# jianwen-xie/Latent-Space-Normalizing-Flow

Measured on AMD Instinct MI355X. Metric: latent-samples/sec through flow+logdet, nz=128 B=65536, higher is better.
Workload: dtype bf16x3; 1 GPU; CIFAR-10 flow prior nz=128 f_width=64 f_depth=5 affine, forward+logdet+log-prob, B=65536 synthetic z per evaluation (BASELINE.json configs[2]); rows_per_gpu=65536, global_rows=65536, parallelism=single GPU, streams=3, clock_ramp_launches_before_warmup=600

## Files before the change

latent-space-normalizing-flow_amd/csrc/lsnf_fwd3p.hip:

```cpp
#include <stdlib.h>
#include <type_traits>
#include "lsnf_l16.h"
#include "lsnf_launch.h"

#if LSNF_L16_PARTS != 3
#error "lsnf_fwd3p.hip is the three-term bf16 kernel"
#endif

#ifndef LSNF_FILLMASK
#define LSNF_FILLMASK 0x7f
#endif

namespace {

struct Fwd3pArgs {
    const float* consts; const float* panels3;
    const float* z_in; const float* objective;
    float* z_out; float* logdet_out; float* ll_out;
    int B, nz, half, n_blocks, vec4;
    double* stats;
    float* hdump; int width;
    float* z_saved; float* act_saved;
    unsigned long long* stamps;
};

#ifdef LSNF_STAMPS
#define P_STAMP(i, INSN)                                                                                \
    do { __builtin_amdgcn_sched_barrier(0);                                                             \
         unsigned long long t_; asm volatile(INSN " %0\n\ts_waitcnt lgkmcnt(0)" : "=s"(t_) :: "memory");  \
         __builtin_amdgcn_sched_barrier(0);                                                             \
         if (a.stamps && lane == 0) a.stamps[(((size_t)blockIdx.x * NWAVES + wave) & 2047) * 64 + (i)] = t_; } while (0)
#else
#define P_STAMP(i, INSN) do {} while (0)
#endif

template <int WT_>
struct Fwd3pCfg : LsnfStackCfg<2, WT_> {
    using S = LsnfStackCfg<2, WT_>;
    static constexpr int F = LSNF_FRAG3_FLOATS;
    static constexpr int OFF3_S2 = F * S::P1 * S::KT1;
    static constexpr int OFF3_S3 = OFF3_S2 + F * S::P2 * S::KT2;
    static constexpr int OFF3_S4 = OFF3_S3 + F * S::P3 * S::KT3;
    static constexpr int BLOCK3 = OFF3_S4 + F * S::P4 * S::KT4;
    static constexpr int SLOT3 = 2 * S::MAXKT * F;
    static constexpr int CONST_FLOATS = S::FWD_CONST;
};

__device__ __forceinline__ void keep(unsigned a, unsigned b, unsigned c) { asm volatile("" :: "v"(a), "v"(b), "v"(c)); }
__device__ __forceinline__ void keep(float a, float b, float c, float d, float e) { asm volatile("" :: "v"(a), "v"(b), "v"(c), "v"(d), "v"(e)); }

struct StepDesc { int acc, tile, s, frag; };
template <int KT> constexpr StepDesc mkstep(int acc, int tl, int in_tile, int kt, int s) { return StepDesc{acc, in_tile, s, ((tl * KT + kt) * 2 + s) * 3}; }

struct Tile16 { f32x4v q[4]; };
struct SplitTile16 { unsigned d[2][3][4]; };

template <int HT, int ST>
__device__ __forceinline__ Tile16 load_tile16(int t, const float* __restrict__ z, const int* rows, int nz, int half, int g, int vw) {
    Tile16 x;
    const int hh = t / HT, tt = t % HT;
#pragma unroll
    for (int ft = 0; ft < 2; ++ft)
#pragma unroll
        for (int st = 0; st < ST; ++st) {
            const int f0 = 32 * tt + l16_feat0(ft, g), col0 = hh * half + f0, q = 2 * ft + st;
            const float* zr = z + (long)rows[st] * (long)nz;
            if (vw == 4) {
                f32x4 v = {0.f, 0.f, 0.f, 0.f};
                if (f0 < half) v = *reinterpret_cast<const f32x4*>(zr + col0);
                x.q[q][0] = v[0]; x.q[q][1] = v[1]; x.q[q][2] = v[2]; x.q[q][3] = v[3];
            } else if (vw == 2) {
                f32x2 v0 = {0.f, 0.f}, v1 = {0.f, 0.f};
                if (f0 < half) v0 = *reinterpret_cast<const f32x2*>(zr + col0);
                if (f0 + 2 < half) v1 = *reinterpret_cast<const f32x2*>(zr + col0 + 2);
                x.q[q][0] = v0[0]; x.q[q][1] = v0[1]; x.q[q][2] = v1[0]; x.q[q][3] = v1[1];
            } else {
#pragma unroll
                for (int j = 0; j < 4; ++j) x.q[q][j] = (f0 + j < half) ? zr[col0 + j] : 0.0f;
            }
        }
    return x;
}
template <int HT, int ST>
__device__ __forceinline__ void store_tile16(int t, const Tile16& x, float* __restrict__ z, const int* rows, const bool* live,
                                             int nz, int half, int g, int vw) {
    const int hh = t / HT, tt = t % HT;
#pragma unroll
    for (int ft = 0; ft < 2; ++ft)
#pragma unroll
        for (int st = 0; st < ST; ++st) {
            if (!live[st]) continue;
            const int f0 = 32 * tt + l16_feat0(ft, g), col0 = hh * half + f0, q = 2 * ft + st;
            float* zr = z + (long)rows[st] * (long)nz;
            if (vw == 4) {
                if (f0 < half) { f32x4 v = {x.q[q][0], x.q[q][1], x.q[q][2], x.q[q][3]}; *reinterpret_cast<f32x4*>(zr + col0) = v; }
            } else if (vw == 2) {
                if (f0 < half) { f32x2 v = {x.q[q][0], x.q[q][1]}; *reinterpret_cast<f32x2*>(zr + col0) = v; }
                if (f0 + 2 < half) { f32x2 v = {x.q[q][2], x.q[q][3]}; *reinterpret_cast<f32x2*>(zr + col0 + 2) = v; }
            } else {
#pragma unroll
                for (int j = 0; j < 4; ++j)
                    if (f0 + j < half) zr[col0 + j] = x.q[q][j];
            }
        }
}
__device__ __forceinline__ const float* bias_lane_ptr(const float* cb, int g) { return cb + (g & 1) * 16 + 4 * (g >> 1); }
__device__ __forceinline__ f32x4v bias_quad(const float* lane_ptr, int float_off) {
    const f32x4 v = *reinterpret_cast<const f32x4*>(lane_ptr + float_off);
    f32x4v r;
#pragma unroll
    for (int j = 0; j < 4; ++j) r[j] = v[j];
    return r;
}
template <class PH> constexpr bool first_touch(int i) {
    for (int j = 0; j < i; ++j)
        if (PH::at(j).acc == PH::at(i).acc && PH::at(j).s == PH::at(i).s) return false;
    return true;
}
template <int ST> __device__ __forceinline__ constexpr int unit_quad(int q) { return ST == 2 ? q : (q & ~1); }
template <int ST> __device__ __forceinline__ constexpr int unit_pair0(int q) { return ST == 2 ? 0 : (q & 1); }
template <int ST> __device__ __forceinline__ constexpr int unit_st(int q) { return ST == 2 ? (q & 1) : 0; }
template <bool RELU, int ST>
__device__ __forceinline__ void split_q16(const Tile16& x, int q, SplitTile16& out) {
#pragma clang fp contract(off)
    const int ft = q >> 1, st = unit_st<ST>(q), qr = unit_quad<ST>(q);
#pragma unroll
    for (int jj = 0; jj < ST; ++jj) {
        const int j = unit_pair0<ST>(q) + jj;
        float a = x.q[qr][2 * j], b = x.q[qr][2 * j + 1];
        if (RELU) { a = fmaxf(a, 0.0f); b = fmaxf(b, 0.0f); }
        const unsigned p1 = pk_bf16(a, b);
        a -= __builtin_bit_cast(float, p1 << 16); b -= __builtin_bit_cast(float, p1 & 0xffff0000u);
        const unsigned p2 = pk_bf16(a, b);
        a -= __builtin_bit_cast(float, p2 << 16); b -= __builtin_bit_cast(float, p2 & 0xffff0000u);
        const int d = 2 * ft + j;
        out.d[st][0][d] = p1; out.d[st][1][d] = p2; out.d[st][2][d] = pk_bf16(a, b);
        keep(out.d[st][0][d], out.d[st][1][d], out.d[st][2][d]);
    }
}
template <int ST>
__device__ __forceinline__ void sigmoid_q16(Tile16& p, int q, float* lsum ) {
    const int st = unit_st<ST>(q), qr = unit_quad<ST>(q), r0 = 2 * unit_pair0<ST>(q);
#pragma unroll
    for (int r = r0; r < r0 + 2 * ST; ++r) {
        float sig, l2;
        lsnf_sigmoid_log2(p.q[qr][r], sig, l2);
        p.q[qr][r] = sig; lsum[st] += l2;
    }
    keep(p.q[qr][r0], p.q[qr][r0 + 1], p.q[qr][r0 + 2 * ST - 2], p.q[qr][r0 + 2 * ST - 1], lsum[st]);
}
template <int ST>
__device__ __forceinline__ void couple_q16(Tile16& v, const Tile16& t, const Tile16& sig, int q) {
    const int qr = unit_quad<ST>(q), r0 = 2 * unit_pair0<ST>(q);
#pragma unroll
    for (int r = r0; r < r0 + 2 * ST; ++r) v.q[qr][r] = (v.q[qr][r] + t.q[qr][r]) * sig.q[qr][r];
}

#ifndef LSNF_STASH_AUX
#define LSNF_STASH_AUX 0
#endif
#ifndef LSNF_STASH_PARTS
#define LSNF_STASH_PARTS 7
#endif
typedef unsigned u32x4s __attribute__((ext_vector_type(4)));
struct StashLane { unsigned zoff, soff, moff, msh, hoff; };
struct StashRsrc { __amdgpu_buffer_rsrc_t r[2]; };
__device__ __forceinline__ StashRsrc stash_rsrc(const float* p, unsigned bytes, unsigned second_off) {
    char* c = reinterpret_cast<char*>(const_cast<float*>(p));
    return StashRsrc{{__builtin_amdgcn_make_buffer_rsrc(c, 0, (int)bytes, 0x00020000),
                      __builtin_amdgcn_make_buffer_rsrc(c + second_off, 0, (int)(bytes > second_off ? bytes - second_off : 0u), 0x00020000)}};
}
template <int HT>
__device__ __forceinline__ void stash_row_quad(const StashRsrc& rs, const StashLane& sl, int t, int q, const Tile16& x, int nz, int half, int g) {
    if constexpr (!(LSNF_STASH_PARTS & 4)) return;
    const int ft = q >> 1, st = q & 1, hh = t / HT, tt = t % HT;
    unsigned off = sl.zoff;
    if (st) off += (unsigned)(16 * nz * 4);
    off = (32 * tt + 16 * ft + 4 * g < half) ? off : 0x80000000u;
    const u32x4s v = __builtin_bit_cast(u32x4s, x.q[q]);
    __builtin_amdgcn_raw_buffer_store_b128(v, rs.r[hh], off + (unsigned)((32 * tt + 16 * ft) * 4), 0, LSNF_STASH_AUX);
}
__device__ __forceinline__ void stash_sigma_quad(const StashRsrc& rs, const StashLane& sl, int t, int q, const Tile16& sg) {
    if constexpr (!(LSNF_STASH_PARTS & 2)) return;
    const int ft = q >> 1, st = q & 1;
    const u32x4s v = __builtin_bit_cast(u32x4s, sg.q[q]);
    __builtin_amdgcn_raw_buffer_store_b128(v, rs.r[t], sl.soff + (unsigned)((2 * ft * 64 + 16 * st) * 16), 0, LSNF_STASH_AUX);
}
__device__ __forceinline__ void mask_q16(const Tile16& h, int q, unsigned (&mk)[2][2]) {
    if constexpr (!(LSNF_STASH_PARTS & 1)) return;
    unsigned m = 0;
#pragma unroll
    for (int r = 3; r >= 0; --r) m = __builtin_amdgcn_alignbit(m, __builtin_bit_cast(unsigned, 0.0f - h.q[q][r]), 31);
    mk[q & 1][q >> 1] = m;
    asm volatile("" :: "v"(m));
}
__device__ __forceinline__ void stash_mask_words(const StashRsrc& rs, const StashLane& sl, int tile, const unsigned (&mk)[2][2]) {
    if constexpr (!(LSNF_STASH_PARTS & 1)) return;
    const unsigned w0 = mk[0][0] | (mk[0][1] << 8), w1 = mk[1][0] | (mk[1][1] << 8);
    unsigned x = ((w0 << 16) | w1) << sl.msh;
    x = lsnf_pair_or32(x);
    __builtin_amdgcn_raw_buffer_store_b32(x >> 16, rs.r[0], sl.moff + (unsigned)(tile * 64 * 4), 0, 0);
    __builtin_amdgcn_raw_buffer_store_b32(x & 0xffffu, rs.r[0], sl.moff + (unsigned)((tile * 64 + 16) * 4), 0, 0);
}
__device__ __forceinline__ void stash_h_quad(const StashRsrc& rs, const StashLane& sl, int t, int q, const Tile16& h, int width) {
    const int ft = q >> 1, st = q & 1;
    f32x4v r;
#pragma unroll
    for (int j = 0; j < 4; ++j) r[j] = fmaxf(h.q[q][j], 0.0f);
    const unsigned off = (32 * t + 16 * ft < width) ? sl.hoff : 0x80000000u;
    __builtin_amdgcn_raw_buffer_store_b128(__builtin_bit_cast(u32x4s, r), rs.r[t], off + (unsigned)((ft * 2 + st) * 1024), 0, LSNF_STASH_AUX);
}

template <int NM, int NV>
__device__ __forceinline__ void pin_mfma() {
    lsnf_static_for<NM>([&](auto mc) {
        constexpr int m = decltype(mc)::value, V = NV / NM + (m < NV % NM ? 1 : 0);
        __builtin_amdgcn_sched_group_barrier(0x008, 1, 0);
        if constexpr (V > 0) __builtin_amdgcn_sched_group_barrier(0x402, V, 0);
    });
}
template <class PH, int ST, class Fill, class Mid>
__device__ __forceinline__ void run_phase16(Tile16* acc, const float* bias_ptr , const SplitTile16* in, const float* lbuf, int lane, Fill&& fill, Mid&& mid) {
    const bf16x8* wp = reinterpret_cast<const bf16x8*>(lbuf) + lane;
    __builtin_amdgcn_sched_barrier(0);
    bf16x8 a[3];
#pragma unroll
    for (int p = 0; p < 3; ++p) a[p] = wp[(PH::at(0).frag + p) * 64];
    f32x4v bq = bias_quad(bias_ptr, 32 * PH::btile(PH::at(0).acc) + 8 * PH::at(0).s);
    __builtin_amdgcn_sched_group_barrier(0x100, 4, 0);
    lsnf_static_for<PH::N>([&](auto ic) {
        constexpr int i = decltype(ic)::value;
        constexpr StepDesc d = PH::at(i);
        mid(ic);
        bf16x8 na[3];
        f32x4v nbq = bq;
#pragma unroll
        for (int p = 0; p < 3; ++p) na[p] = a[p];
        if constexpr (i + 1 < PH::N) {
#pragma unroll
            for (int p = 0; p < 3; ++p) na[p] = wp[(PH::at(i + 1).frag + p) * 64];
            if constexpr (first_touch<PH>(i + 1)) nbq = bias_quad(bias_ptr, 32 * PH::btile(PH::at(i + 1).acc) + 8 * PH::at(i + 1).s);
        }
#ifndef LSNF_ABL_NOFILL
        fill(ic);
#endif
        const SplitTile16& x = in[d.tile];
        constexpr bool first = first_touch<PH>(i);
#define LSNF_Q_MMA(WI, XI) \
        acc[d.acc].q[2 * d.s + 0] = __builtin_amdgcn_mfma_f32_16x16x32_bf16(a[WI], __builtin_bit_cast(bf16x8, u32x4{x.d[0][XI][0], x.d[0][XI][1], x.d[0][XI][2], x.d[0][XI][3]}), (first && WI == 2 && XI == 0) ? bq : acc[d.acc].q[2 * d.s + 0], 0, 0, 0); \
        if constexpr (ST == 2) acc[d.acc].q[2 * d.s + 1] = __builtin_amdgcn_mfma_f32_16x16x32_bf16(a[WI], __builtin_bit_cast(bf16x8, u32x4{x.d[1][XI][0], x.d[1][XI][1], x.d[1][XI][2], x.d[1][XI][3]}), (first && WI == 2 && XI == 0) ? bq : acc[d.acc].q[2 * d.s + 1], 0, 0, 0);
#ifdef LSNF_ABL_NOMFMA
        LSNF_Q_MMA(0, 0)
#else
        LSNF_F3_TERMS(LSNF_Q_MMA)
#endif
#undef LSNF_Q_MMA
        if constexpr (i + 1 < PH::N) __builtin_amdgcn_sched_group_barrier(0x100, first_touch<PH>(i + 1) ? 4 : 3, 0);
        pin_mfma<6 * ST, (PH::valu(i) * ST) / 2>();
        __builtin_amdgcn_sched_barrier(0);
#pragma unroll
        for (int p = 0; p < 3; ++p) a[p] = na[p];
        bq = nbq;
    });
}

struct QhNoStores { static constexpr int stores(int) { return 0; } };
struct QhS1a : QhNoStores {
    static constexpr int N = 16;
    static constexpr int btile(int acc) { return acc; }
    static constexpr StepDesc at(int i) { return mkstep<4>((i >> 1) & 1, (i >> 1) & 1, i >> 2, i >> 2, i & 1); }
    static constexpr int valu(int i) { return i < 2 ? 22 : (i < 6 ? 28 : (i < 8 ? 16 : (i < 12 ? 22 : 0))); }
};
struct QhS1b : QhNoStores {
    static constexpr int N = 16;
    static constexpr int btile(int acc) { return 2 + acc; }
    static constexpr StepDesc at(int i) { return mkstep<4>((i >> 1) & 1, (i >> 1) & 1, i >> 2, i >> 2, i & 1); }
    static constexpr int valu(int i) { return i >= 8 ? 22 : 0; }
};
struct QhS23 : QhNoStores {
    static constexpr int N = 16;
    static constexpr int btile(int acc) { return 4 + acc; }
    static constexpr StepDesc at(int i) {
        if (i < 8) { const int tl = i >> 2, kt = (i >> 1) & 1; return mkstep<2>(tl, tl, kt, kt, i & 1); }
        const int j = i - 8, kt = j >> 2, tl = (j >> 1) & 1;
        return mkstep<2>(2 + tl, 2 + tl, 2 + kt, kt, j & 1);
    }
    static constexpr int valu(int i) { return (i >= 4 && i < 12) ? 26 : (i >= 13 ? 26 : 0); }
};
struct QhS4 : QhNoStores {
    static constexpr int N = 16;
    static constexpr int btile(int acc) { return 8 + (acc == 0 ? 2 : (acc == 1 ? 0 : (acc == 2 ? 3 : 1))); }
    static constexpr int torder(int j) { return j == 0 ? 2 : (j == 1 ? 0 : (j == 2 ? 3 : 1)); }
    static constexpr StepDesc at(int i) { const int kt = i >> 3, j = (i >> 1) & 3; return mkstep<2>(j, torder(j), kt, kt, i & 1); }
    static constexpr int valu(int i) { return i < 4 ? 26 : (i < 9 ? 0 : (i < 12 ? 28 : (i == 12 ? 36 : (i == 13 ? 24 : 22)))); }
};

struct QsS1a : QhS1a {
    static constexpr int valu(int i) { return (i == 6 || i == 7) ? 20 : (i >= 8 && i < 12 ? 23 : QhS1a::valu(i)); }
    static constexpr int stores(int i) { return (i >= 2 && i < 6) ? 1 : ((i == 6 || i == 7) ? 2 : (i >= 8 && i < 12 ? 1 : 0)); }
};
struct QsS1b : QhS1b {
    static constexpr int valu(int i) { return i < 8 ? (i >= 6 ? 1 : 0) : (i < 14 ? 23 : 22); }
    static constexpr int stores(int i) { return (i >= 6 && i < 14) ? 1 : 0; }
};
struct QsS23 : QhS23 {
    static constexpr int valu(int i) { return (i >= 4 && i < 12) ? (i == 8 ? 44 : 34) : (i >= 13 ? 34 : 0); }
    static constexpr int stores(int i) { return i == 8 ? 2 : 0; }
};
struct QsS4 : QhS4 {
    static constexpr int valu(int i) { return i < 4 ? 34 : ((i >= 6 && i < 9) ? 10 + QhS4::valu(i) : QhS4::valu(i)); }
    static constexpr int stores(int i) { return (i >= 6 && i < 9) ? 2 : ((i >= 9 && i < 13) ? 1 : 0); }
};
struct QxS23 : QsS23 {
    static constexpr int valu(int i) { return QsS23::valu(i) + (((i >= 4 && i < 12) || i >= 13) ? 2 : 0); }
    static constexpr int stores(int i) { return QsS23::stores(i) + (((i >= 4 && i < 12) || i >= 13) ? 1 : 0); }
};
struct QxS4 : QsS4 {
    static constexpr int valu(int i) { return QsS4::valu(i) + (i < 4 ? 2 : 0); }
    static constexpr int stores(int i) { return QsS4::stores(i) + (i < 4 ? 1 : 0); }
};
template <class PH> constexpr int stores_after(int last_dma_step) {
    int n = 0;
    for (int i = last_dma_step + 1; i < PH::N; ++i) n += PH::stores(i);
    return n;
}

template <int WT, int NWAVES, int ST, int STASH = 0>
__global__ __launch_bounds__(64 * NWAVES, 1) void lsnf_fwd3q_kernel(const Fwd3pArgs a) {
    static_assert(!STASH || ST == 2, "the stash tile is a wave's 32 rows");
    using TS1a = std::conditional_t<STASH != 0, QsS1a, QhS1a>;
    using TS1b = std::conditional_t<STASH != 0, QsS1b, QhS1b>;
    using TS23 = std::conditional_t<STASH == 2, QxS23, std::conditional_t<STASH != 0, QsS23, QhS23>>;
    using TS4 = std::conditional_t<STASH == 2, QxS4, std::conditional_t<STASH != 0, QsS4, QhS4>>;
    using C = Fwd3pCfg<WT>;
    static_assert(WT == 2, "lsnf_fwd3q_kernel: f_width <= 64 instantiation");
    constexpr int THREADS = 64 * NWAVES;
    constexpr int HT = 2, NZT = 4, F = C::F;
    constexpr int SLOT = C::SLOT3;
    extern __shared__ __attribute__((aligned(16))) float smem[];
    float* cst = smem;
    float* const buf0 = smem + a.n_blocks * C::CONST_FLOATS;
    const int tid = threadIdx.x;
    const int wave = __builtin_amdgcn_readfirstlane(tid >> 6);
    const int lane = tid & 63;
    const int n = lane & 15, g = lane >> 4;
    P_STAMP(0, "s_memtime");
    P_STAMP(50, "s_memrealtime");
    const int n_phases = 4 * a.n_blocks;
    auto phase_src = [&](int k) -> const float* {
        const float* gb = a.panels3 + (size_t)(k >> 2) * C::BLOCK3;
        const int j = k & 3;
        return gb + (j == 0 ? 0 : (j == 1 ? 2 * 4 * F : (j == 2 ? C::OFF3_S2 : C::OFF3_S4)));
    };
    auto sync_issue = [&](int k, auto left) {
#ifdef LSNF_ABL_SKIPSYNC
        if ((LSNF_ABL_SKIPSYNC >> (k & 3)) & 1) return;
#endif
        asm volatile("s_waitcnt vmcnt(%0)" :: "n"(decltype(left)::value) : "memory");
        __syncthreads();
#ifdef LSNF_FWD3Q_BURST_DMA
        if (k + 1 < n_phases) issue_kib<48, NWAVES>(phase_src(k + 1), buf0 + ((k + 1) & 1) * SLOT, wave, lane);
#endif
    };
    constexpr int PER_WAVE = 48 / NWAVES, EVERY = STASH ? 1 : 16 / PER_WAVE, LAST_DMA = (PER_WAVE - 1) * EVERY;
    using Left0 = std::integral_constant<int, 0>;
    using LeftS1a = std::integral_constant<int, stores_after<TS1a>(LAST_DMA)>;
    using LeftS1b = std::integral_constant<int, stores_after<TS1b>(LAST_DMA)>;
    using LeftS23 = std::integral_constant<int, stores_after<TS23>(LAST_DMA) + (STASH == 2 ? 1 : 0)>;
    using LeftS4 = std::integral_constant<int, stores_after<TS4>(LAST_DMA)>;
    const float* dma_src = nullptr; float* dma_dst = nullptr;
    auto dma_arm = [&](int k) {
        dma_src = phase_src(k + 1 < n_phases ? k + 1 : k);
        dma_dst = buf0 + ((k + 1) & 1) * SLOT;
    };
    auto dma_step = [&](auto ic) {
#ifndef LSNF_FWD3Q_BURST_DMA
        constexpr int i = decltype(ic)::value;
        if constexpr (i % EVERY == 0 && i / EVERY < PER_WAVE) issue_piece<NWAVES>(dma_src, dma_dst, i / EVERY, wave, lane);
#endif
    };

    const int wbase = (blockIdx.x * NWAVES + wave) * (16 * ST);
    int sample[2] = {0, 0}, rows[2] = {0, 0}; bool live[2] = {false, false};
#pragma unroll
    for (int st = 0; st < ST; ++st) { sample[st] = wbase + 16 * st + n; live[st] = sample[st] < a.B; rows[st] = live[st] ? sample[st] : a.B - 1; }

    Tile16 v[NZT];
    SplitTile16 xs[NZT];
    Tile16 p1, t1;
    float lsum[2] = {0.0f, 0.0f};
    {
        const Tile16 x0 = load_tile16<HT, ST>(0, a.z_in, rows, a.nz, a.half, g, a.vec4);
        const Tile16 x1 = load_tile16<HT, ST>(1, a.z_in, rows, a.nz, a.half, g, a.vec4);
        v[2] = load_tile16<HT, ST>(2, a.z_in, rows, a.nz, a.half, g, a.vec4);
        v[3] = load_tile16<HT, ST>(3, a.z_in, rows, a.nz, a.half, g, a.vec4);
        __builtin_amdgcn_sched_barrier(0);
        issue_kib<48, NWAVES>(phase_src(0), buf0, wave, lane);
        for (int i = tid; i < a.n_blocks * C::CONST_FLOATS; i += THREADS) cst[i] = a.consts[i];
#pragma unroll
        for (int q = 0; q < 4; ++q) { split_q16<false, ST>(x0, q, xs[0]); split_q16<false, ST>(x1, q, xs[1]); }
        split_q16<false, ST>(v[2], 0, xs[2]); split_q16<false, ST>(v[2], 1, xs[2]);
#pragma unroll
        for (int q = 0; q < 4; ++q)
#pragma unroll
            for (int r = 0; r < 4; ++r) { p1.q[q][r] = 80.0f; t1.q[q][r] = 0.0f; }
    }
    float ell[2];
#pragma unroll
    for (int st = 0; st < 2; ++st) ell[st] = (st < ST && a.objective) ? a.objective[rows[st]] : 0.0f;
    float ss01[2] = {0.0f, 0.0f};
    StashLane sl0 = {0u, 0u, 0u, 0u};
    const LsnfActLayout al = lsnf_act_layout(a.B, HT, WT);
    const unsigned zbytes = (unsigned)a.B * (unsigned)a.nz * 4u, abytes = (unsigned)(al.per_block * 4);
    if constexpr (STASH) {
        const unsigned tile_byte = (unsigned)(wbase >> 5) * (unsigned)(al.per_tile * 4), L = (unsigned)(n + 32 * (g & 1));
        sl0.zoff = ((unsigned)(wbase + n) * (unsigned)a.nz + 4u * g) * 4u;
        sl0.soff = tile_byte + ((unsigned)(g >> 1) * 64u + L) * 16u;
        sl0.moff = tile_byte + (unsigned)(al.mask_off * 4) + L * 4u;
        sl0.msh = 4u * (g >> 1);
        sl0.hoff = (unsigned)(wbase >> 5) * (unsigned)(32 * a.width * 4) + (unsigned)(n * 4 + g) * 16u;
    }
    const LsnfDumpLayout dl = lsnf_dump_layout(a.B, a.nz, a.width);
    const unsigned hbytes = (unsigned)(((size_t)a.B + 31) / 32 * 32 * a.width * 4);
    sync_issue(0, Left0{});
    P_STAMP(1, "s_memtime");

    for (int blk = 0; blk < a.n_blocks; ++blk) {
        const float* cb = cst + blk * C::CONST_FLOATS;
        const bool more = blk + 1 < a.n_blocks;
        const int k0 = 4 * blk;
        SplitTile16 vh[4];
        SplitTile16 h2s[WT];
        Tile16 hh[4], tp[4];
        const bool zs = STASH && a.z_saved != nullptr, as = STASH && a.act_saved != nullptr;
        const float* zc = more ? (zs ? a.z_saved + (size_t)blk * a.B * a.nz : a.z_out) : a.z_out;
        const float* zp = blk > 0 ? (zs ? a.z_saved + (size_t)(blk - 1) * a.B * a.nz : a.z_out) : a.z_out;
        const StashRsrc rs_zc = stash_rsrc(zc, (more && !zs) ? 0u : zbytes, (unsigned)a.half * 4u);
        const StashRsrc rs_zp = stash_rsrc(zp, (blk > 0 && !zs) ? 0u : zbytes, (unsigned)a.half * 4u);
        const StashRsrc rs_ac = stash_rsrc(as ? a.act_saved + (size_t)blk * al.per_block : a.z_out, as ? abytes : 0u, 4096u);
        const StashRsrc rs_ap = stash_rsrc(as ? a.act_saved + (size_t)(blk > 0 ? blk - 1 : 0) * al.per_block : a.z_out, as ? abytes : 0u, 4096u);
        StashLane sl = sl0;
        if constexpr (STASH) asm volatile("" : "+v"(sl.zoff), "+v"(sl.soff), "+v"(sl.moff));
        if constexpr (STASH == 2) asm volatile("" : "+v"(sl.hoff));
        const float* hd = (STASH == 2) ? a.hdump + (size_t)blk * dl.per_block : a.z_out;
        const StashRsrc rs_h1 = stash_rsrc(STASH == 2 ? hd + dl.off_h1 : hd, STASH == 2 ? hbytes : 0u, 4096u);
        const StashRsrc rs_h2 = stash_rsrc(STASH == 2 ? hd + dl.off_h2 : hd, STASH == 2 ? hbytes : 0u, 4096u);
        unsigned mk1[2][2], mk2[2][2], mk3[2][2];

        if (blk == 1) P_STAMP(10, "s_memtime");
        {
            const float* bv = bias_lane_ptr(cb, g);
            if (k0 > 0) sync_issue(k0, LeftS4{});
            dma_arm(k0);
            run_phase16<TS1a, ST>(v, bv, xs, buf0 + (k0 & 1) * SLOT, lane, [&](auto ic) {
                constexpr int i = decltype(ic)::value;
                if constexpr (STASH && i >= 8 && i < 12) stash_row_quad<HT>(rs_zp, sl, 2, i - 8, v[2], a.nz, a.half, g);
                if constexpr (i < 2) split_q16<false, ST>(v[2], 2 + i, xs[2]);
                else if constexpr (i < 6) {
                    sigmoid_q16<ST>(p1, i - 2, lsum);
                    if constexpr (STASH) stash_sigma_quad(rs_ap, sl, 1, i - 2, p1);
                } else if constexpr (i < 8) {
                    couple_q16<ST>(v[3], t1, p1, 2 * (i - 6)); couple_q16<ST>(v[3], t1, p1, 2 * (i - 6) + 1);
                    if constexpr (STASH) { stash_row_quad<HT>(rs_zp, sl, 3, 2 * (i - 6), v[3], a.nz, a.half, g); stash_row_quad<HT>(rs_zp, sl, 3, 2 * (i - 6) + 1, v[3], a.nz, a.half, g); }
                } else if constexpr (i < 12) split_q16<false, ST>(v[3], i - 8, xs[3]);
            }, dma_step);
        }
        if (blk == 1) P_STAMP(11, "s_memtime");
        {
            const float* bv = bias_lane_ptr(cb, g);
            sync_issue(k0 + 1, LeftS1a{});
            dma_arm(k0 + 1);
            run_phase16<TS1b, ST>(v + 2, bv, xs, buf0 + ((k0 + 1) & 1) * SLOT, lane, [&](auto ic) {
                constexpr int i = decltype(ic)::value;
                if constexpr (STASH && i >= 6 && i < 14) stash_row_quad<HT>(rs_zc, sl, (i - 6) >> 2, (i - 6) & 3, v[(i - 6) >> 2], a.nz, a.half, g);
                if constexpr (i >= 8) split_q16<false, ST>(v[(i - 8) >> 2], i & 3, vh[(i - 8) >> 2]);
            }, dma_step);
        }
        if (blk == 1) P_STAMP(12, "s_memtime");
        if (!more) {
            int ln = lane;
            asm volatile("" : "+v"(ln));
            const int smp[2] = {wbase + (ln & 15), wbase + 16 + (ln & 15)};
#pragma unroll
            for (int t = 0; t < HT; ++t) {
                if constexpr (!STASH) store_tile16<HT, ST>(t, v[t], a.z_out, smp, live, a.nz, a.half, g, a.vec4);
#pragma unroll
                for (int ft = 0; ft < 2; ++ft)
#pragma unroll
                    for (int st = 0; st < ST; ++st)
#pragma unroll
                        for (int r = 0; r < 4; ++r) ss01[st] += v[t].q[2 * ft + st][r] * v[t].q[2 * ft + st][r];
            }
        }
#pragma unroll
        for (int st = 0; st < 2; ++st) { ell[st] = ell[st] + cb[32 * C::NP + 0]; ell[st] = ell[st] + cb[32 * C::NP + 1]; }
        {
            static_assert(C::P1 == 4 && C::P2 == 2 && C::P3 == 2, "bias tile indices of the phase tables");
            const float* bv = bias_lane_ptr(cb, g);
            sync_issue(k0 + 2, LeftS1b{});
            dma_arm(k0 + 2);
            run_phase16<TS23, ST>(hh, bv, vh, buf0 + ((k0 + 2) & 1) * SLOT, lane, [&](auto ic) {
                constexpr int i = decltype(ic)::value;
                if constexpr (i >= 4 && i < 8) split_q16<true, ST>(hh[0], i - 4, vh[2]);
                if constexpr (i >= 8 && i < 12) split_q16<true, ST>(hh[1], i - 8, vh[3]);
                if constexpr (i >= 13) split_q16<true, ST>(hh[2], i - 13, h2s[0]);
                if constexpr (STASH) {
                    if constexpr (i >= 4 && i < 8) mask_q16(hh[0], i - 4, mk3);
                    if constexpr (i == 8) stash_mask_words(rs_ac, sl, 0, mk3);
                    if constexpr (i >= 8 && i < 12) mask_q16(hh[1], i - 8, mk1);
                    if constexpr (i >= 13) mask_q16(hh[2], i - 13, mk2);
                }
                if constexpr (STASH == 2) {
                    if constexpr (i >= 4 && i < 8) stash_h_quad(rs_h1, sl, 0, i - 4, hh[0], a.width);
                    if constexpr (i >= 8 && i < 12) stash_h_quad(rs_h1, sl, 1, i - 8, hh[1], a.width);
                    if constexpr (i >= 13) stash_h_quad(rs_h2, sl, 0, i - 13, hh[2], a.width);
                }
            }, dma_step);
        }
        if (blk == 1) P_STAMP(13, "s_memtime");
        xs[0] = vh[0]; xs[1] = vh[1];
        {
            constexpr int B4 = C::P1 + C::P2 + C::P3;
            static_assert(B4 == 8, "bias tile indices of the phase tables");
            const float* bv = bias_lane_ptr(cb, g);
            split_q16<true, ST>(hh[2], 3, h2s[0]);
            if constexpr (STASH) mask_q16(hh[2], 3, mk2);
            if constexpr (STASH == 2) stash_h_quad(rs_h2, sl, 0, 3, hh[2], a.width);
            sync_issue(k0 + 3, LeftS23{});
            dma_arm(k0 + 3);
            run_phase16<TS4, ST>(tp, bv, h2s, buf0 + ((k0 + 3) & 1) * SLOT, lane, [&](auto ic) {
                constexpr int i = decltype(ic)::value;
                if constexpr (i < 4) split_q16<true, ST>(hh[3], i, h2s[1]);
                if constexpr (STASH) {
                    if constexpr (i < 4) mask_q16(hh[3], i, mk3);
                    if constexpr (i == 6) stash_mask_words(rs_ac, sl, 1, mk1);
                    if constexpr (i == 7) stash_mask_words(rs_ac, sl, WT + 0, mk2);
                    if constexpr (i == 8) stash_mask_words(rs_ac, sl, WT + 1, mk3);
                }
                if constexpr (STASH == 2 && i < 4) stash_h_quad(rs_h2, sl, 1, i, hh[3], a.width);
                if constexpr (i >= 9 && i < 13) { sigmoid_q16<ST>(tp[0], i - 9, lsum); if constexpr (STASH) stash_sigma_quad(rs_ac, sl, 0, i - 9, tp[0]); }
                if constexpr (i == 12) couple_q16<ST>(v[2], tp[1], tp[0], 0);
                if constexpr (i == 13) { couple_q16<ST>(v[2], tp[1], tp[0], 1); couple_q16<ST>(v[2], tp[1], tp[0], 2); couple_q16<ST>(v[2], tp[1], tp[0], 3); }
                if constexpr (i >= 14) split_q16<false, ST>(v[2], i - 14, xs[2]);
            }, dma_step);
            p1 = tp[2]; t1 = tp[3];
        }
        if (blk == 1) P_STAMP(14, "s_memtime");
    }
    P_STAMP(40, "s_memtime");
#pragma unroll
    for (int q = 0; q < 4; ++q) { sigmoid_q16<ST>(p1, q, lsum); couple_q16<ST>(v[3], t1, p1, q); }
    if constexpr (STASH) {
        const bool as = a.act_saved != nullptr;
        const StashRsrc rs_al = stash_rsrc(as ? a.act_saved + (size_t)(a.n_blocks - 1) * al.per_block : a.z_out, as ? abytes : 0u, 4096u);
#pragma unroll
        for (int q = 0; q < 4; ++q) stash_sigma_quad(rs_al, sl0, 1, q, p1);
    }
#pragma unroll
    for (int st = 0; st < ST; ++st) ell[st] = ell[st] + -0.6931471805599453f * l16_group_sum(lsum[st]);

    float ss[2] = {ss01[0], ss01[1]};
    int ln_e = lane;
    asm volatile("" : "+v"(ln_e));
    const int smp_e[2] = {wbase + (ln_e & 15), wbase + 16 + (ln_e & 15)};
#pragma unroll
    for (int t = HT; t < NZT; ++t) {
#pragma unroll
        for (int ft = 0; ft < 2; ++ft)
#pragma unroll
            for (int st = 0; st < ST; ++st)
#pragma unroll
                for (int r = 0; r < 4; ++r) ss[st] += v[t].q[2 * ft + st][r] * v[t].q[2 * ft + st][r];
        store_tile16<HT, ST>(t, v[t], a.z_out, smp_e, live, a.nz, a.half, g, a.vec4);
    }
    float ll[2] = {0.0f, 0.0f};
#pragma unroll
    for (int st = 0; st < ST; ++st) {
        ll[st] = (-0.5f * l16_group_sum(ss[st]) + 1.8378770664093453f) + ell[st];
        if (live[st] && g == 0) {
            const int smp = smp_e[st];
            a.logdet_out[smp] = ell[st];
            if (a.ll_out) a.ll_out[smp] = ll[st];
        }
    }
    asm volatile("s_waitcnt vmcnt(0)" ::: "memory");
    if (a.stats) {
        double dl = 0.0, dd = 0.0;
#pragma unroll
        for (int st = 0; st < ST; ++st)
            if (live[st] && g == 0) { dl += (double)ll[st]; dd += (double)ell[st]; }
#pragma unroll
        for (int o = 8; o > 0; o >>= 1) { dl += __shfl_xor(dl, o, 64); dd += __shfl_xor(dd, o, 64); }
        __syncthreads();
        double* red = reinterpret_cast<double*>(buf0);
        if (lane == 0) { red[2 * wave] = dl; red[2 * wave + 1] = dd; }
        __syncthreads();
        if (wave == 0) {
            double tl = 0.0, td = 0.0;
            for (int w = 0; w < NWAVES; ++w) { tl += red[2 * w]; td += red[2 * w + 1]; }
            lsnf_publish_stats(a.stats, tl, td, a.B, lane);
        }
    }
    P_STAMP(41, "s_memtime");
    P_STAMP(51, "s_memrealtime");
}

size_t fwd3q_lds(int n_blocks) {
    using C = Fwd3pCfg<2>;
    return ((size_t)n_blocks * C::CONST_FLOATS + 2 * (size_t)C::SLOT3) * sizeof(float);
}

template <int WT, int NWAVES, int ST, int STASH = 0>
hipError_t launch_fwd3q_w(const Fwd3pArgs& a, hipStream_t stream) {
    return lsnf_launch_kernel<lsnf_fwd3q_kernel<WT, NWAVES, ST, STASH>>(lsnf_grid(a.B, 16 * ST * NWAVES), 64 * NWAVES, fwd3q_lds(a.n_blocks), stream, a);
}
}

bool lsnf_forward3q_covers(const LsnfForwardCall& c) {
    const LsnfGeo& g = c.g;
    if (g.HT != 2 || g.WT != 2 || fwd3q_lds(c.n_blocks) > 160 * 1024) return false;
    if (c.hdump && (!c.hdump_tiled || !c.act_saved || (c.n_blocks > 1 && !c.z_saved) || c.first_block != 0 || (g.width & 15) ||
                    ((size_t)c.B + 32) * g.width * 4 >= (1ull << 31))) return false;
    const bool stash = c.act_saved != nullptr || c.z_saved != nullptr;
    return !(stash && (c.vec4 != 4 || (size_t)c.B * g.nz * 4 >= (1ull << 31) || lsnf_act_layout(c.B, g.HT, g.WT).per_block * 4 >= (1ull << 31) ||
                       (((size_t)c.act_saved | (size_t)c.z_saved | (size_t)c.z_out) & 15)));
}

hipError_t lsnf_launch_forward3q(const LsnfForwardCall& c) {
    if (!lsnf_forward3q_covers(c)) return hipErrorInvalidValue;
    const bool stash = c.act_saved != nullptr || c.z_saved != nullptr;
    const hipStream_t stream = c.stream;
    Fwd3pArgs a;
    lsnf_fill_forward(a, c);
    a.panels3 = lsnf_f3b_panels_at(c);
    a.hdump = c.hdump; a.width = c.g.width;
    a.stamps = lsnf_stamps_buffer();
    static const char* shape = getenv("LSNF_FWD3Q_SHAPE");
    const int sh = shape ? atoi(shape) : (c.B > 128 * 256 ? 82 : (c.B > 64 * 256 ? 81 : 41));
    if (c.hdump) return (sh == 82) ? launch_fwd3q_w<2, 8, 2, 2>(a, stream) : launch_fwd3q_w<2, 4, 2, 2>(a, stream);
    if (stash) return (sh == 82) ? launch_fwd3q_w<2, 8, 2, 1>(a, stream) : launch_fwd3q_w<2, 4, 2, 1>(a, stream);
    if (sh == 82) return launch_fwd3q_w<2, 8, 2>(a, stream);
    if (sh == 42) return launch_fwd3q_w<2, 4, 2>(a, stream);
    if (sh == 81) return launch_fwd3q_w<2, 8, 1>(a, stream);
    return launch_fwd3q_w<2, 4, 1>(a, stream);
}
```

Baseline: 757.3 million latent-samples/s.

## Add CU-sharing forward variant with half-phase LDS buffers for two workgroups per CU

Adds a PAIR form of the three-term forward kernel: 4 waves, launch bounds allowing two workgroups per CU, and a single weight slot split into two half-phase buffers, so the LDS footprint fits in half a CU. Each phase runs as two half-phases over remapped fragment subsets, each wave streaming its own 6 KiB chunk, with a barrier between halves. It becomes the default for large batches when the plain forward path is used. The aim is to let a second workgroup hide DMA and barrier stalls, at the cost of an extra barrier per phase and tighter register limits.

```diff
diff --git a/latent-space-normalizing-flow_amd/csrc/lsnf_fwd3p.hip b/latent-space-normalizing-flow_amd/csrc/lsnf_fwd3p.hip
--- a/latent-space-normalizing-flow_amd/csrc/lsnf_fwd3p.hip
+++ b/latent-space-normalizing-flow_amd/csrc/lsnf_fwd3p.hip
@@ -9,6 +9,13 @@
 
 #ifndef LSNF_FILLMASK
 #define LSNF_FILLMASK 0x7f
+#endif
+
+#ifndef LSNF_PAIR_DMA_PER_STEP
+#define LSNF_PAIR_DMA_PER_STEP 6
+#endif
+#ifndef LSNF_FWD3Q_LARGE
+#define LSNF_FWD3Q_LARGE 242
 #endif
 
 namespace {
@@ -112,11 +119,15 @@
     for (int j = 0; j < 4; ++j) r[j] = v[j];
     return r;
 }
-template <class PH> constexpr bool first_touch(int i) {
-    for (int j = 0; j < i; ++j)
-        if (PH::at(j).acc == PH::at(i).acc && PH::at(j).s == PH::at(i).s) return false;
-    return true;
-}
+template <class PH> struct FirstTouch {
+    static constexpr bool at(int i) {
+        for (int j = 0; j < i; ++j)
+            if (PH::at(j).acc == PH::at(i).acc && PH::at(j).s == PH::at(i).s) return false;
+        return true;
+    }
+};
+template <class PH> constexpr bool first_touch(int i) { return FirstTouch<PH>::at(i); }
+template <class T> struct TypeTag { using type = T; };
 template <int ST> __device__ __forceinline__ constexpr int unit_quad(int q) { return ST == 2 ? q : (q & ~1); }
 template <int ST> __device__ __forceinline__ constexpr int unit_pair0(int q) { return ST == 2 ? 0 : (q & 1); }
 template <int ST> __device__ __forceinline__ constexpr int unit_st(int q) { return ST == 2 ? (q & 1) : 0; }
@@ -325,9 +336,69 @@
     return n;
 }
 
-template <int WT, int NWAVES, int ST, int STASH = 0>
-__global__ __launch_bounds__(64 * NWAVES, 1) void lsnf_fwd3q_kernel(const Fwd3pArgs a) {
+struct PairMap {
+    static constexpr int src(int kind, int h, int c) {
+        constexpr int T[3][2][4] = {{{0, 1, 4, 5}, {2, 3, 6, 7}}, {{0, 1, 2, 3}, {4, 5, 6, 7}}, {{0, 2, 4, 6}, {1, 3, 5, 7}}};
+        return T[kind][h][c];
+    }
+    static constexpr int kind(int j) { return j < 2 ? 0 : j - 1; }
+    static constexpr unsigned packed(int kind, int h) {
+        unsigned v = 0;
+        for (int c = 0; c < 4; ++c) v |= (unsigned)src(kind, h, c) << (4 * c);
+        return v;
+    }
+    static constexpr int compact(int kind, int h, int chunk) {
+        for (int c = 0; c < 4; ++c)
+            if (src(kind, h, c) == chunk) return c;
+        return -1;
+    }
+    static constexpr bool once(int kind) {
+        for (int chunk = 0; chunk < 8; ++chunk) {
+            int n = 0;
+            for (int h = 0; h < 2; ++h)
+                for (int c = 0; c < 4; ++c) n += src(kind, h, c) == chunk;
+            if (n != 1) return false;
+        }
+        return true;
+    }
+};
+static_assert(PairMap::once(0) && PairMap::once(1) && PairMap::once(2), "the piece tables cover every fragment of a panel exactly once");
+template <class PH, int KIND, int H>
+struct HalfPh {
+    static constexpr int N = 8;
+    static constexpr int btile(int acc) { return PH::btile(acc); }
+    static constexpr StepDesc at(int i) {
+        StepDesc d = PH::at(8 * H + i);
+        d.frag = (PairMap::compact(KIND, H, d.frag / 6) * 2 + d.s) * 3;
+        return d;
+    }
+    static constexpr int valu(int i) { return PH::valu(8 * H + i); }
+    static constexpr int stores(int i) { return PH::stores(8 * H + i); }
+    static constexpr bool resident() {
+        for (int i = 0; i < N; ++i)
+            if (PairMap::compact(KIND, H, PH::at(8 * H + i).frag / 6) < 0) return false;
+        return true;
+    }
+};
+template <class PH, int KIND, int H> struct FirstTouch<HalfPh<PH, KIND, H>> {
+    static constexpr bool at(int i) { return FirstTouch<PH>::at(8 * H + i); }
+};
+static_assert(HalfPh<QhS1a, 0, 0>::resident() && HalfPh<QhS1a, 0, 1>::resident() && HalfPh<QhS1b, 0, 0>::resident() && HalfPh<QhS1b, 0, 1>::resident() &&
+              HalfPh<QhS23, 1, 0>::resident() && HalfPh<QhS23, 1, 1>::resident() && HalfPh<QhS4, 2, 0>::resident() && HalfPh<QhS4, 2, 1>::resident(),
+              "the step order of a half-phase stays inside its four fragments");
+__device__ __forceinline__ void issue_piece_at(const float* __restrict__ gsrc, float* lbuf, int kib, int lane) {
+    const char* sb = reinterpret_cast<const char*>(gsrc) + (size_t)kib * 1024u;
+    const unsigned m0v = (unsigned)(size_t)((LSNF_AS3 char*)lbuf) + (unsigned)kib * 1024u;
+    const unsigned lane_off = (unsigned)lane * 16u;
+    unsigned keep_m0;
+    asm volatile("s_mov_b32 %0, m0\n\ts_mov_b32 m0, %3\n\ts_nop 0\n\tglobal_load_lds_dwordx4 %1, %2\n\ts_mov_b32 m0, %0"
+                 : "=&s"(keep_m0) : "v"(lane_off), "s"(sb), "s"(m0v) : "memory");
+}
+
+template <int WT, int NWAVES, int ST, int STASH = 0, int PAIR = 0>
+__global__ __launch_bounds__(64 * NWAVES, PAIR ? 2 : 1) void lsnf_fwd3q_kernel(const Fwd3pArgs a) {
     static_assert(!STASH || ST == 2, "the stash tile is a wave's 32 rows");
+    static_assert(!PAIR || (STASH == 0 && NWAVES == 4 && ST == 2), "the CU-sharing form: plain forward, one wave per SIMD and workgroup, 32 rows per wave");
     using TS1a = std::conditional_t<STASH != 0, QsS1a, QhS1a>;
     using TS1b = std::conditional_t<STASH != 0, QsS1b, QhS1b>;
     using TS23 = std::conditional_t<STASH == 2, QxS23, std::conditional_t<STASH != 0, QsS23, QhS23>>;
@@ -337,6 +408,9 @@
     constexpr int THREADS = 64 * NWAVES;
     constexpr int HT = 2, NZT = 4, F = C::F;
     constexpr int SLOT = C::SLOT3;
+    constexpr int HSLOT = SLOT / 2;
+    static_assert(HSLOT == 4 * F && (2 * HSLOT + 5 * C::CONST_FLOATS) * sizeof(float) <= 80 * 1024,
+                  "PAIR: two half-phase buffers and the constants of the five-block stack in half a CU's LDS");
     extern __shared__ __attribute__((aligned(16))) float smem[];
     float* cst = smem;
     float* const buf0 = smem + a.n_blocks * C::CONST_FLOATS;
@@ -359,6 +433,7 @@
         asm volatile("s_waitcnt vmcnt(%0)" :: "n"(decltype(left)::value) : "memory");
         __syncthreads();
 #ifdef LSNF_FWD3Q_BURST_DMA
+        static_assert(!PAIR, "the burst-DMA timing build fills whole 48 KiB buffers: the CU-sharing form has none");
         if (k + 1 < n_phases) issue_kib<48, NWAVES>(phase_src(k + 1), buf0 + ((k + 1) & 1) * SLOT, wave, lane);
 #endif
     };
@@ -376,8 +451,41 @@
     auto dma_step = [&](auto ic) {
 #ifndef LSNF_FWD3Q_BURST_DMA
         constexpr int i = decltype(ic)::value;
-        if constexpr (i % EVERY == 0 && i / EVERY < PER_WAVE) issue_piece<NWAVES>(dma_src, dma_dst, i / EVERY, wave, lane);
-#endif
+        if constexpr (PAIR) {
+            constexpr int PS = LSNF_PAIR_DMA_PER_STEP;
+            if constexpr (i * PS < 6) {
+#pragma unroll
+                for (int s = i * PS; s < i * PS + PS && s < 6; ++s) issue_piece_at(dma_src, dma_dst, s, lane);
+            }
+        } else if constexpr (i % EVERY == 0 && i / EVERY < PER_WAVE) issue_piece<NWAVES>(dma_src, dma_dst, i / EVERY, wave, lane);
+#endif
+    };
+    auto pair_chunk = [&](unsigned packed) { return (int)((packed >> (4 * wave)) & 7u); };
+    auto pair_arm = [&](auto jc, auto hc, int k) {
+        constexpr int J = decltype(jc)::value, H = decltype(hc)::value;
+        if constexpr (H == 0) {
+            dma_src = phase_src(k) + pair_chunk(PairMap::packed(PairMap::kind(J), 1)) * F;
+            dma_dst = buf0 + HSLOT + wave * F;
+        } else {
+            const bool last = k + 1 >= n_phases;
+            dma_src = phase_src(last ? k : k + 1) + pair_chunk(last ? PairMap::packed(PairMap::kind(J), 1) : PairMap::packed(PairMap::kind((J + 1) & 3), 0)) * F;
+            dma_dst = buf0 + wave * F;
+        }
+    };
+    auto run_phase = [&](auto ph, auto jc, int k, Tile16* acc, const float* bv, const SplitTile16* in, auto&& fill) {
+        using PH = typename decltype(ph)::type;
+        if constexpr (!PAIR) {
+            dma_arm(k);
+            run_phase16<PH, ST>(acc, bv, in, buf0 + (k & 1) * SLOT, lane, fill, dma_step);
+        } else {
+            constexpr int KIND = PairMap::kind(decltype(jc)::value);
+            pair_arm(jc, std::integral_constant<int, 0>{}, k);
+            run_phase16<HalfPh<PH, KIND, 0>, ST>(acc, bv, in, buf0, lane, fill, dma_step);
+            sync_issue(k, Left0{});
+            pair_arm(jc, std::integral_constant<int, 1>{}, k);
+            run_phase16<HalfPh<PH, KIND, 1>, ST>(acc, bv, in, buf0 + HSLOT, lane,
+                                                 [&](auto ic) { fill(std::integral_constant<int, decltype(ic)::value + 8>{}); }, dma_step);
+        }
     };
 
     const int wbase = (blockIdx.x * NWAVES + wave) * (16 * ST);
@@ -395,7 +503,11 @@
         v[2] = load_tile16<HT, ST>(2, a.z_in, rows, a.nz, a.half, g, a.vec4);
         v[3] = load_tile16<HT, ST>(3, a.z_in, rows, a.nz, a.half, g, a.vec4);
         __builtin_amdgcn_sched_barrier(0);
-        issue_kib<48, NWAVES>(phase_src(0), buf0, wave, lane);
+        if constexpr (PAIR) {
+            const float* src0 = phase_src(0) + pair_chunk(PairMap::packed(0, 0)) * F;
+#pragma unroll
+            for (int s = 0; s < 6; ++s) issue_piece_at(src0, buf0 + wave * F, s, lane);
+        } else issue_kib<48, NWAVES>(phase_src(0), buf0, wave, lane);
         for (int i = tid; i < a.n_blocks * C::CONST_FLOATS; i += THREADS) cst[i] = a.consts[i];
 #pragma unroll
         for (int q = 0; q < 4; ++q) { split_q16<false, ST>(x0, q, xs[0]); split_q16<false, ST>(x1, q, xs[1]); }
@@ -451,8 +563,7 @@
         {
             const float* bv = bias_lane_ptr(cb, g);
             if (k0 > 0) sync_issue(k0, LeftS4{});
-            dma_arm(k0);
-            run_phase16<TS1a, ST>(v, bv, xs, buf0 + (k0 & 1) * SLOT, lane, [&](auto ic) {
+            run_phase(TypeTag<TS1a>{}, std::integral_constant<int, 0>{}, k0, v, bv, xs, [&](auto ic) {
                 constexpr int i = decltype(ic)::value;
                 if constexpr (STASH && i >= 8 && i < 12) stash_row_quad<HT>(rs_zp, sl, 2, i - 8, v[2], a.nz, a.half, g);
                 if constexpr (i < 2) split_q16<false, ST>(v[2], 2 + i, xs[2]);
@@ -463,18 +574,17 @@
                     couple_q16<ST>(v[3], t1, p1, 2 * (i - 6)); couple_q16<ST>(v[3], t1, p1, 2 * (i - 6) + 1);
                     if constexpr (STASH) { stash_row_quad<HT>(rs_zp, sl, 3, 2 * (i - 6), v[3], a.nz, a.half, g); stash_row_quad<HT>(rs_zp, sl, 3, 2 * (i - 6) + 1, v[3], a.nz, a.half, g); }
                 } else if constexpr (i < 12) split_q16<false, ST>(v[3], i - 8, xs[3]);
-            }, dma_step);
+            });
         }
         if (blk == 1) P_STAMP(11, "s_memtime");
         {
             const float* bv = bias_lane_ptr(cb, g);
             sync_issue(k0 + 1, LeftS1a{});
-            dma_arm(k0 + 1);
-            run_phase16<TS1b, ST>(v + 2, bv, xs, buf0 + ((k0 + 1) & 1) * SLOT, lane, [&](auto ic) {
+            run_phase(TypeTag<TS1b>{}, std::integral_constant<int, 1>{}, k0 + 1, v + 2, bv, xs, [&](auto ic) {
                 constexpr int i = decltype(ic)::value;
                 if constexpr (STASH && i >= 6 && i < 14) stash_row_quad<HT>(rs_zc, sl, (i - 6) >> 2, (i - 6) & 3, v[(i - 6) >> 2], a.nz, a.half, g);
                 if constexpr (i >= 8) split_q16<false, ST>(v[(i - 8) >> 2], i & 3, vh[(i - 8) >> 2]);
-            }, dma_step);
+            });
         }
         if (blk == 1) P_STAMP(12, "s_memtime");
         if (!more) {
@@ -498,8 +608,7 @@
             static_assert(C::P1 == 4 && C::P2 == 2 && C::P3 == 2, "bias tile indices of the phase tables");
             const float* bv = bias_lane_ptr(cb, g);
             sync_issue(k0 + 2, LeftS1b{});
-            dma_arm(k0 + 2);
-            run_phase16<TS23, ST>(hh, bv, vh, buf0 + ((k0 + 2) & 1) * SLOT, lane, [&](auto ic) {
+            run_phase(TypeTag<TS23>{}, std::integral_constant<int, 2>{}, k0 + 2, hh, bv, vh, [&](auto ic) {
                 constexpr int i = decltype(ic)::value;
                 if constexpr (i >= 4 && i < 8) split_q16<true, ST>(hh[0], i - 4, vh[2]);
                 if constexpr (i >= 8 && i < 12) split_q16<true, ST>(hh[1], i - 8, vh[3]);
@@ -515,7 +624,7 @@
                     if constexpr (i >= 8 && i < 12) stash_h_quad(rs_h1, sl, 1, i - 8, hh[1], a.width);
                     if constexpr (i >= 13) stash_h_quad(rs_h2, sl, 0, i - 13, hh[2], a.width);
                 }
-            }, dma_step);
+            });
         }
         if (blk == 1) P_STAMP(13, "s_memtime");
         xs[0] = vh[0]; xs[1] = vh[1];
@@ -527,8 +636,7 @@
             if constexpr (STASH) mask_q16(hh[2], 3, mk2);
             if constexpr (STASH == 2) stash_h_quad(rs_h2, sl, 0, 3, hh[2], a.width);
             sync_issue(k0 + 3, LeftS23{});
-            dma_arm(k0 + 3);
-            run_phase16<TS4, ST>(tp, bv, h2s, buf0 + ((k0 + 3) & 1) * SLOT, lane, [&](auto ic) {
+            run_phase(TypeTag<TS4>{}, std::integral_constant<int, 3>{}, k0 + 3, tp, bv, h2s, [&](auto ic) {
                 constexpr int i = decltype(ic)::value;
                 if constexpr (i < 4) split_q16<true, ST>(hh[3], i, h2s[1]);
                 if constexpr (STASH) {
@@ -542,7 +650,7 @@
                 if constexpr (i == 12) couple_q16<ST>(v[2], tp[1], tp[0], 0);
                 if constexpr (i == 13) { couple_q16<ST>(v[2], tp[1], tp[0], 1); couple_q16<ST>(v[2], tp[1], tp[0], 2); couple_q16<ST>(v[2], tp[1], tp[0], 3); }
                 if constexpr (i >= 14) split_q16<false, ST>(v[2], i - 14, xs[2]);
-            }, dma_step);
+            });
             p1 = tp[2]; t1 = tp[3];
         }
         if (blk == 1) P_STAMP(14, "s_memtime");
@@ -605,14 +713,14 @@
     P_STAMP(51, "s_memrealtime");
 }
 
-size_t fwd3q_lds(int n_blocks) {
+size_t fwd3q_lds(int n_blocks, bool pair = false) {
     using C = Fwd3pCfg<2>;
-    return ((size_t)n_blocks * C::CONST_FLOATS + 2 * (size_t)C::SLOT3) * sizeof(float);
-}
-
-template <int WT, int NWAVES, int ST, int STASH = 0>
+    return ((size_t)n_blocks * C::CONST_FLOATS + (pair ? 1 : 2) * (size_t)C::SLOT3) * sizeof(float);
+}
+
+template <int WT, int NWAVES, int ST, int STASH = 0, int PAIR = 0>
 hipError_t launch_fwd3q_w(const Fwd3pArgs& a, hipStream_t stream) {
-    return lsnf_launch_kernel<lsnf_fwd3q_kernel<WT, NWAVES, ST, STASH>>(lsnf_grid(a.B, 16 * ST * NWAVES), 64 * NWAVES, fwd3q_lds(a.n_blocks), stream, a);
+    return lsnf_launch_kernel<lsnf_fwd3q_kernel<WT, NWAVES, ST, STASH, PAIR>>(lsnf_grid(a.B, 16 * ST * NWAVES), 64 * NWAVES, fwd3q_lds(a.n_blocks, PAIR), stream, a);
 }
 }
 
@@ -636,9 +744,12 @@
     a.hdump = c.hdump; a.width = c.g.width;
     a.stamps = lsnf_stamps_buffer();
     static const char* shape = getenv("LSNF_FWD3Q_SHAPE");
-    const int sh = shape ? atoi(shape) : (c.B > 128 * 256 ? 82 : (c.B > 64 * 256 ? 81 : 41));
+    const bool pair_ok = !c.hdump && !stash && fwd3q_lds(c.n_blocks, true) <= 80 * 1024;
+    int sh = shape ? atoi(shape) : (c.B > 128 * 256 ? LSNF_FWD3Q_LARGE : (c.B > 64 * 256 ? 81 : 41));
+    if (sh == 242 && !pair_ok) sh = 82;
     if (c.hdump) return (sh == 82) ? launch_fwd3q_w<2, 8, 2, 2>(a, stream) : launch_fwd3q_w<2, 4, 2, 2>(a, stream);
     if (stash) return (sh == 82) ? launch_fwd3q_w<2, 8, 2, 1>(a, stream) : launch_fwd3q_w<2, 4, 2, 1>(a, stream);
+    if (sh == 242) return launch_fwd3q_w<2, 4, 2, 0, 1>(a, stream);
     if (sh == 82) return launch_fwd3q_w<2, 8, 2>(a, stream);
     if (sh == 42) return launch_fwd3q_w<2, 4, 2>(a, stream);
     if (sh == 81) return launch_fwd3q_w<2, 8, 1>(a, stream);
```

Result: faster. 770.3 million latent-samples/s (median of 6 runs) (+1.7%).
